# inkandswitch/peritext

Measured on NVIDIA H100. Metric: ops merged/sec across batch, higher is better.
Workload: dtype u32

## Files before the change

### peritext_b200/csrc/engine.cu

```cuda
#include <algorithm>
#include <atomic>
#include <cstdlib>
#include <cstring>
#include <initializer_list>
#include <string>
#include <thread>
#include <utility>
#include <vector>

#include "merge_kernel.cuh"
#include "warp_kernel.cuh"
#include "patch_kernel.cuh"
#include "patch_large_kernel.cuh"
#include "team_kernel.cuh"
#include "render_kernel.cuh"
#include "patch_json_kernel.cuh"
#include "append_kernel.cuh"
#include "change_kernel.cuh"
#include "exchange_kernel.cuh"
#include "changes_json_kernel.cuh"
#include "upload_kernel.cuh"
#include "scan_kernel.cuh"
#include "admit_kernel.cuh"
#include "query_kernel.cuh"
// ... 70 lines not shown
    uint64_t n_insdel = 0, n_mark = 0;
    std::vector<pt_log_desc> h_desc;
    ptp::Plan plan;
    DevBuf d_runs, d_tokens, d_run_off, d_tok_off, d_cins, d_cmarks;
    DevBuf d_desc, d_insdel, d_marks, d_order, d_counters, d_results, d_text_off, d_span_off, d_text, d_spans, d_pool, d_slab, d_retry, d_seq;
    DevBuf d_bsum, d_ctoff, d_csoff, d_ctext, d_cspans;
    DevBuf d_cdesc, d_changes, d_deps, d_admit;
    std::vector<pt_change_desc> h_cdesc;
    uint64_t n_changes = 0, n_deps = 0;
    DevBuf d_patch_recs, d_patch_items, d_patch_status;
    DevBuf d_patch_first;
    DevBuf d_large_cand, d_large_scratch;
    HostBuf h_patch_recs, h_patch_items, h_patch_status, h_patch_misc, h_patch_first;
    DevBuf d_jval, d_jvoff, d_jlink, d_jloff, d_jcom, d_jcoff;
    JsonBufs spans_json, patches_json;
    JsonBufs changes_json;
    HostBuf h_cj_status;
    DevBuf d_picnt, d_piseg, d_pibsum, d_pitmp, d_pisorted;
    uint64_t patch_cap = 0;
    bool have_changes = false;
    uint32_t adm_maxR = 1;
    const pt_insdel_rec* dp_insdel = nullptr;
    const pt_mark_rec* dp_marks = nullptr;
    DevBuf d_half_insdel, d_half_marks;
    HostBuf h_stage, h_results, h_text, h_spans, h_pool, h_misc, h_seq, h_ctoff, h_csoff;
    HostBuf h_chg_status, h_chg_desc, h_chg_insdel, h_chg_marks;
    HostBuf h_xch_totals, h_xch_status, h_xch_off, h_xch_delivered, h_xch_desc;
    bool have_actors = false;
    DevBuf d_anames, d_aoff, d_afirst;
    std::vector<uint64_t> h_afirst, h_abyte;
    std::vector<char> h_adense;
    HostBuf h_act_data, h_act_off, h_act_first;
    HostBuf h_syn_totals, h_syn_status, h_syn_off, h_syn_aoff, h_syn_amap;
    HostBuf h_add_totals, h_add_rank, h_add_aoff, h_add_amap;
    cudaEvent_t ev0 = nullptr, ev1 = nullptr;
    cudaStream_t side = nullptr, launch_stream = nullptr;
    cudaEvent_t ev_fork = nullptr, ev_join = nullptr;
    uint64_t launches = 0;
    cudaGraphExec_t graph_exec = nullptr;
    bool graph_ok = false, graph_tried = false;
    uint32_t merges_since_upload = 0;
    bool dl_begun = false;
    uint32_t kernels_per_merge = 0;
    uint64_t pool_used_host = 0;
};

namespace {
// ... 188 lines not shown
int install_plan(pt_batch* b, const pt_packed_ops& ops, ptp::Plan&& plan, bool own_records) {
    b->n_logs = ops.n_logs; b->n_insdel = ops.n_insdel_total; b->n_mark = ops.n_mark_total;
    b->h_desc.assign(ops.logs, ops.logs + ops.n_logs);
    b->plan = std::move(plan);
    int rc;
    if ((rc = alloc_and_upload_plan(b))) return rc;
    if (own_records) {
        if ((rc = reserve_n<pt_insdel_rec>(b->d_insdel, b->n_insdel))) return rc;
        if ((rc = reserve_n<pt_mark_rec>(b->d_marks, b->n_mark))) return rc;
    }
    return PT_OK;
}

int begin_upload(pt_batch* b, const pt_packed_ops& ops, bool own_records) {
    PT_CUDA(cudaSetDevice(b->device));
    PT_CUDA(cudaStreamSynchronize(b->stream));
    b->have_batch = false; b->merged = false; b->dl_begun = false; b->have_changes = false; b->have_actors = false;
    drop_graph(b);
    ptp::Plan plan;
    if (const char* err = ptp::make_plan(ops, b->limits, b->num_sms, plan)) { g_last_error = err; return PT_ERR_INVALID; }
    return install_plan(b, ops, std::move(plan), own_records);
}

int derive_half_records(pt_batch* b) {
    const uint32_t* nr = b->plan.n_route;
    if (!(nr[ptp::kPacked3] + nr[ptp::kCompact] + nr[ptp::kDirect])) { b->d_half_insdel.release(); b->d_half_marks.release(); return PT_OK; }
    int rc;
    if ((rc = reserve_n<uint2>(b->d_half_insdel, b->n_insdel)) || (rc = reserve_n<uint4>(b->d_half_marks, b->n_mark))) return rc;
    const uint64_t total = b->n_insdel + b->n_mark;
    const uint32_t threads = 256;
    if (total) {
        ptu::derive_half_records_kernel<<<warp_grid(b, total, threads, 1), threads, 0, b->stream>>>(
            b->dp_insdel, b->dp_marks, (uint2*)b->d_half_insdel.p, (uint4*)b->d_half_marks.p, b->n_insdel, b->n_mark);
        PT_CUDA(launched(b));
    }
    return PT_OK;
}

int finish_upload(pt_batch* b, const void* insdel, const void* marks, std::initializer_list<std::pair<const void*, uint64_t>> sources) {
    bool pageable = false;
    for (const auto& s : sources) {
        if (!s.second) continue;
        cudaPointerAttributes a;
        if (cudaPointerGetAttributes(&a, s.first) != cudaSuccess) { cudaGetLastError(); pageable = true; }
        else if (a.type != cudaMemoryTypeHost) pageable = true;
    }
    b->dp_insdel = (const pt_insdel_rec*)insdel; b->dp_marks = (const pt_mark_rec*)marks;
    int rc;
    if ((rc = derive_half_records(b))) return rc;
    if (pageable) PT_CUDA(cudaStreamSynchronize(b->stream));
    b->have_batch = true;
    return PT_OK;
}

template <class Q, class A, class Launch>
int run_queries(pt_batch* b, const char* fn, const char* verb, const Q* queries, uint32_t n, A* out, Launch launch) {
    if (!b || (n && (!queries || !out))) return PT_ERR_INVALID;
    if (!b->merged) { g_last_error = std::string(verb) + " before merge"; return PT_ERR_STATE; }
    if (!(b->limits.flags & PT_FLAG_EMIT_SEQUENCE)) { g_last_error = "the handle was created without PT_FLAG_EMIT_SEQUENCE"; return PT_ERR_STATE; }
    if (!n) return PT_OK;
    PT_CUDA(cudaSetDevice(b->device));
    DevBuf dq, da;
    int rc;
    if ((rc = dq.reserve((size_t)n * sizeof(Q))) || (rc = da.reserve((size_t)n * sizeof(A)))) return rc;
    cudaError_t e = cudaMemcpyAsync(dq.p, queries, (size_t)n * sizeof(Q), cudaMemcpyHostToDevice, b->stream);
    if (e == cudaSuccess) {
        launch(warp_grid(b, n, 128), 128u, (const Q*)dq.p, (A*)da.p);
        e = launched(b);
    }
    if (e == cudaSuccess) e = cudaMemcpyAsync(out, da.p, (size_t)n * sizeof(A), cudaMemcpyDeviceToHost, b->stream);
    if (e == cudaSuccess) e = cudaStreamSynchronize(b->stream);
    if (e != cudaSuccess) { g_last_error = std::string(fn) + ": " + cudaGetErrorString(e); return PT_ERR_CUDA; }
// ... 423 lines not shown
            pta::splice_changes_kernel<<<warp_grid(b, n, threads), threads, 0, b->stream>>>(
                (const pt_change_desc*)b->d_cdesc.p, (const pt_change_desc*)ncdesc.p, (const pt_change_desc*)dcdesc.p, n, DR,
                (const pt_change_rec*)b->d_changes.p, (const pt_dep_rec*)b->d_deps.p, d_dchg, d_ddep, (pt_change_rec*)nch.p, (pt_dep_rec*)ndp.p);
            PT_CUDA(launched(b));
        }
    }
    uint32_t bad = 0;
    PT_CUDA(cudaMemcpyAsync(&bad, abad.p, 4, cudaMemcpyDeviceToHost, b->stream));
    PT_CUDA(cudaStreamSynchronize(b->stream));
    if (bad) { g_last_error = std::string(fn) + "a resident comment rank is outside comment_map"; return PT_ERR_INVALID; }
    bool keep_actors = !(R.actor_off && R.actor_off[n] > R.actor_off[0]) && !(R.ctr_off && R.ctr_off[n] > R.ctr_off[0]);
    for (uint32_t i = 0; keep_actors && i < n; i++) keep_actors = nd[i].n_actors == b->h_desc[i].n_actors;
    b->have_actors = b->have_actors && keep_actors;
    b->have_batch = false; b->merged = false; b->dl_begun = false;
    drop_graph(b);
    b->d_insdel.swap(nins); b->d_marks.swap(nmarks);
    if (dch) {
        b->d_cdesc.swap(ncdesc); b->d_changes.swap(nch); b->d_deps.swap(ndp);
        b->h_cdesc = std::move(ncd); b->n_changes = n_ch; b->n_deps = n_dp; b->adm_maxR = maxR;
    }
    if ((rc = install_plan(b, ops, std::move(plan), true))) return rc;
    PT_CUDA(cudaStreamSynchronize(b->stream));
    b->dp_insdel = (const pt_insdel_rec*)b->d_insdel.p; b->dp_marks = (const pt_mark_rec*)b->d_marks.p;
    if ((rc = derive_half_records(b))) return rc;
    b->have_batch = true;
    return PT_OK;
}

int pt_batch_append(pt_batch* b, const pt_packed_ops* delta, const pt_append_remap* remap, const pt_change_table* dch) {
    if (!b || !delta || (delta->n_logs && !delta->logs)) return PT_ERR_INVALID;
    if (!b->have_batch) { g_last_error = "pt_batch_append before pt_batch_upload"; return PT_ERR_STATE; }
    return splice_append(b, "pt_batch_append: ", delta, false, remap ? *remap : pt_append_remap{}, dch, false);
}

static std::string check_change(const pt_batch* b, const pt_change_input& in, std::vector<pt_log_desc>& dd, std::vector<uint32_t>& new_elems,
                                std::vector<uint32_t>& work) {
    const uint32_t n = b->n_logs;
    if (in.n_logs != n) return "the input has " + std::to_string(in.n_logs) + " logs and the batch " + std::to_string(n);
    if (!n) return std::string();
    if (!in.actor || !in.input_off) return "null actor or input_off";
    if (in.input_off[0] != 0) return "input_off[0] is not 0";
    if ((in.input_off[n] && !in.ops) || (in.n_tokens && !in.tokens)) return "null ops or tokens with a nonzero count";
    dd.resize(n); new_elems.assign(n, 0);
    uint64_t io = 0, mo = 0;
    for (uint32_t i = 0; i < n; i++) {
        const pt_log_desc& L = b->h_desc[i];
        const uint64_t lo = in.input_off[i], hi = in.input_off[i + 1];
// ... 564 lines not shown
    } else {
        for (uint32_t i = 0; i < n; i++) tot[i] = pty::SyncTotals{};
    }
    if ((rc = grow_tables(b, fn, grow, tot, n, (const uint8_t*)ddata.p, (const unsigned long long*)doff.p, (const unsigned long long*)dfirst.p,
                          (const unsigned long long*)dnew.p, b->h_add_aoff, b->h_add_amap, &spliced))) return rc;
    if (count) {
        const pty::Tables T{(const uint8_t*)b->d_anames.p, (const unsigned long long*)b->d_aoff.p, (const unsigned long long*)b->d_afirst.p};
        pty::add_ranks_kernel<<<warp_grid(b, n, 128), 128, 0, b->stream>>>(n, T, (const uint8_t*)ddata.p, (const unsigned long long*)doff.p,
                                                                           (const unsigned long long*)dfirst.p, (uint16_t*)drank.p);
        PT_CUDA(launched(b));
        PT_CUDA(cudaMemcpyAsync(b->h_add_rank.p, drank.p, count * 2, cudaMemcpyDeviceToHost, b->stream));
        PT_CUDA(cudaStreamSynchronize(b->stream));
    }
    *out = pt_actor_view{n, count, (const uint16_t*)b->h_add_rank.p, (const uint64_t*)b->h_add_aoff.p, (const uint16_t*)b->h_add_amap.p, spliced ? 1u : 0u};
    return PT_OK;
}

static int enqueue_merge(pt_batch* b) {
    DevCounters* c = counters(b);
    PT_CUDA(cudaMemsetAsync(c, 0, sizeof(DevCounters), b->stream));
    ptk::BatchParams P{};
    P.desc = (const pt_log_desc*)b->d_desc.p;
    P.insdel = b->dp_insdel; P.marks = b->dp_marks;
    P.half_insdel = (const uint2*)b->d_half_insdel.p; P.half_marks = (const uint4*)b->d_half_marks.p;
    P.results = (pt_log_result*)b->d_results.p;
    P.text_off = (const uint64_t*)b->d_text_off.p; P.span_off = (const uint64_t*)b->d_span_off.p;
    P.text = (uint32_t*)b->d_text.p; P.spans = (pt_span*)b->d_spans.p;
    P.comment_pool = (uint32_t*)b->d_pool.p; P.comment_used = &c->comment_used; P.comment_cap = b->plan.pool_cap;
    P.slab = (char*)b->d_slab.p;
    P.slab_counter = c->slab; P.slab_slots = b->plan.slab_slots;
    P.seq = (b->limits.flags & PT_FLAG_EMIT_SEQUENCE) ? (uint32_t*)b->d_seq.p : nullptr;
    P.stats = c->stats;
    P.admit = nullptr;
    if (b->have_changes && b->n_logs) {
        const auto [wpb, smem] = actor_shape(b->adm_maxR);
        if (smem > 48 * 1024) PT_CUDA(cudaFuncSetAttribute(ptadm::admit_kernel, cudaFuncAttributeMaxDynamicSharedMemorySize, (int)smem));
        ptadm::admit_kernel<<<warp_grid(b, b->n_logs, wpb * 32), wpb * 32, smem, b->stream>>>(
            (const pt_change_desc*)b->d_cdesc.p, (const pt_change_rec*)b->d_changes.p, (const pt_dep_rec*)b->d_deps.p, (const pt_log_desc*)b->d_desc.p,
            b->n_logs, b->adm_maxR, (uint32_t*)b->d_admit.p, (pt_log_result*)b->d_results.p);
        PT_CUDA(launched(b));
        P.admit = (const uint32_t*)b->d_admit.p;
    }
    { const char* e = getenv("PT_PREFETCH"); P.prefetch_next = e ? (uint32_t)atoi(e) : 0u; }
    { const char* e = getenv("PT_WARP_FLAGS"); P.warp_flags = e ? (uint32_t)atoi(e) : 0x704u; }
    { const char* e = getenv("PT_TMA"); P.use_tma = e ? (uint32_t)atoi(e) : 1u; }
    int rc;
    const uint32_t* bin_first = b->plan.bin_first;
// ... 588 lines not shown
```

### peritext_b200/csrc/merge_kernel.cuh

```cuda
#pragma once
#include <cuda_runtime.h>
#include <stdint.h>

#include "../../include/peritext_b200.h"
#include "../../include/pt_digest.h"

namespace ptk {

struct BatchParams {
    const pt_log_desc* __restrict__ desc;
    const pt_insdel_rec* __restrict__ insdel;
    const pt_mark_rec* __restrict__ marks;
    const uint2* __restrict__ half_insdel;
    const uint4* __restrict__ half_marks;
    const uint32_t* __restrict__ order;
    uint32_t n_work;
    uint32_t* work_counter;
    pt_log_result* results;
    const uint64_t* __restrict__ text_off;
    const uint64_t* __restrict__ span_off;
    uint32_t* text;
    pt_span* spans;
    uint32_t* comment_pool;
    unsigned long long* comment_used;
    unsigned long long comment_cap;
    char* slab;
    unsigned long long slab_bytes;
    uint32_t* slab_counter;
    uint32_t slab_slots;
    uint32_t smem_arena_bytes;
    unsigned long long* stats;
    uint32_t* retry_list;
    uint32_t* retry_count;
    const uint32_t* n_work_dev;
    uint32_t prefetch_next;
    uint32_t warp_flags;
    uint32_t use_tma;
// ... 975 lines not shown
```

### peritext_b200/csrc/upload_kernel.cuh

```cuda
#pragma once
#include <cstdint>

#include "../../include/peritext_b200.h"

namespace ptu {

__global__ void expand_runs_kernel(const pt_log_desc* __restrict__ desc, const unsigned long long* __restrict__ run_off,
                                   const unsigned long long* __restrict__ tok_off, const pt_run_rec* __restrict__ runs,
                                   const uint32_t* __restrict__ tokens, pt_insdel_rec* __restrict__ out, uint32_t n_logs) {
    const uint32_t warp = (blockIdx.x * blockDim.x + threadIdx.x) >> 5, lane = threadIdx.x & 31, nwarps = (gridDim.x * blockDim.x) >> 5;
    for (uint32_t li = warp; li < n_logs; li += nwarps) {
        const unsigned long long r0 = run_off[li], r1 = run_off[li + 1];
        pt_insdel_rec* o = out + desc[li].insdel_off;
        const uint32_t* tk = tokens + tok_off[li];
        uint32_t rec_base = 0, tok_base = 0;
        for (unsigned long long rb = r0; rb < r1; rb += 32) {
            const unsigned long long ri = rb + lane;
            uint4 r = make_uint4(0, 0, 0, 0);
            uint32_t cnt = 0, kind = 0;
            if (ri < r1) { r = __ldg(reinterpret_cast<const uint4*>(runs + ri)); cnt = r.w & 0x3FFFFFFFu; kind = r.w >> 30; }
            uint32_t tcnt = kind == PT_KIND_INSERT ? cnt : 0u;
            uint32_t pr = cnt, pt = tcnt;
#pragma unroll
            for (int d = 1; d < 32; d <<= 1) { uint32_t a = __shfl_up_sync(0xffffffffu, pr, d), b2 = __shfl_up_sync(0xffffffffu, pt, d); if (lane >= (uint32_t)d) { pr += a; pt += b2; } }
// ... 21 lines not shown
    for (unsigned long long i = (unsigned long long)blockIdx.x * blockDim.x + threadIdx.x; i < n; i += (unsigned long long)gridDim.x * blockDim.x) {
        const uint2 q = __ldg(reinterpret_cast<const uint2*>(in + i));
        const uint32_t tok22 = q.y >> 10;
        uint4 o;
        o.x = q.x & 0xFFFFu; o.y = q.x >> 16;
        o.z = (q.y & 0xFu) | (((q.y >> 4) & 0xFu) << 16);
        o.w = (((q.y >> 8) & 3u) << 30) | ((tok22 & 0x200000u) ? PT_TOKEN_POOLED : 0u) | (tok22 & 0x1FFFFFu);
        reinterpret_cast<uint4*>(out)[i] = o;
    }
}
__global__ void expand_mark_c16_kernel(const pt_mark_c16* __restrict__ in, pt_mark_rec* __restrict__ out, unsigned long long n) {
    for (unsigned long long i = (unsigned long long)blockIdx.x * blockDim.x + threadIdx.x; i < n; i += (unsigned long long)gridDim.x * blockDim.x) {
        const uint4 q = __ldg(reinterpret_cast<const uint4*>(in + i));
        uint4 a, b;
        a.x = q.x & 0xFFFFu;
        a.y = (q.w & 0xFu) | (((q.w >> 12) & 7u) << 16) | (((q.w >> 15) & 0xFu) << 24);
        a.z = q.x >> 16; a.w = q.y & 0xFFFFu;
        b.x = ((q.w >> 4) & 0xFu) | (((q.w >> 8) & 0xFu) << 16);
        b.y = q.z; b.z = q.y >> 16; b.w = 0;
        reinterpret_cast<uint4*>(out)[2 * i] = a; reinterpret_cast<uint4*>(out)[2 * i + 1] = b;
    }
}

__device__ __forceinline__ uint32_t sat16(uint32_t v) { return min(v, 0xFFFFu); }
__device__ __forceinline__ uint32_t sat8(uint32_t v) { return min(v, 0xFFu); }
__global__ void derive_half_records_kernel(const pt_insdel_rec* __restrict__ ins, const pt_mark_rec* __restrict__ mk,
                                           uint2* __restrict__ hins, uint4* __restrict__ hmk, unsigned long long n, unsigned long long m) {
    for (unsigned long long i = (unsigned long long)blockIdx.x * blockDim.x + threadIdx.x; i < n + m; i += (unsigned long long)gridDim.x * blockDim.x) {
        if (i < n) {
            const uint4 r = __ldg(reinterpret_cast<const uint4*>(ins + i));
            hins[i] = make_uint2(sat16(r.x) | (sat16(r.y) << 16), sat8(r.z & 0xFFFFu) | (sat8(r.z >> 16) << 8) | ((r.w >> 30) << 16));
        } else {
            const uint4* q = reinterpret_cast<const uint4*>(mk + (i - n));
            const uint4 a = __ldg(q), b = __ldg(q + 1);
            hmk[i - n] = make_uint4(sat16(a.x) | (sat16(a.z) << 16), sat16(a.w) | (sat16(b.z) << 16), b.y,
                                    sat8(a.y & 0xFFFFu) | (sat8(b.x & 0xFFFFu) << 8) | (sat8(b.x >> 16) << 16) |
                                        (((a.y >> 16) & 7u) << 24) | (((a.y >> 24) & 0xFu) << 27));
        }
    }
}

}
```

### peritext_b200/csrc/warp_kernel.cuh

```cuda
#pragma once
#include "merge_kernel.cuh"

namespace ptk {

constexpr uint32_t kFull = 0xffffffffu;
constexpr uint32_t kNone16 = 0xFFFFu;
constexpr uint32_t kWarpGrab = 4;
constexpr uint32_t kMaxSegSurvivorWork = 1536;
constexpr uint32_t kMaxCommentSurvivors = 48;

__device__ __forceinline__ uint32_t warp_incl_scan(uint32_t v, uint32_t lane) {
#pragma unroll
    for (int o = 1; o < 32; o <<= 1) { const uint32_t y = __shfl_up_sync(kFull, v, o); if (lane >= (uint32_t)o) v += y; }
    return v;
}

struct WArena {
    uint32_t base, used, cap;
    template <class T> __device__ __forceinline__ T* alloc(uint32_t count) {
        const uint32_t off = used;
        used += (uint32_t)((count * sizeof(T) + 15u) & ~15u);
        return reinterpret_cast<T*>(ptk_smem + base + off);
    }
    __device__ __forceinline__ bool fits() const { return used <= cap; }
// ... 38 lines not shown
    __device__ __forceinline__ void mark(int k) { const long long now = clock64(); c[k] += (unsigned long long)(now - t); t = now; }
};
#define PT_PHASE(k) pclk.mark(k)
#define PT_PHASE_PARAM , PhaseClock& pclk
#define PT_PHASE_ARG , pclk
#else
#define PT_PHASE(k) ((void)0)
#define PT_PHASE_PARAM
#define PT_PHASE_ARG
#endif

constexpr int kIdDirect = 0, kIdCompact = 1, kIdPacked3 = 2;

template <int IDM>
__device__ __forceinline__ int warp_merge_one_log(const BatchParams& P, const uint32_t li, const uint32_t slice_base, const uint32_t slice_bytes, const uint32_t li_next, PhaseSync ps PT_PHASE_PARAM) {
    const uint32_t lane = threadIdx.x & 31u;
    const uint32_t lt = (1u << lane) - 1u;

    const uint4 dsc0 = __ldg(reinterpret_cast<const uint4*>(P.desc + li)), dsc1 = __ldg(reinterpret_cast<const uint4*>(P.desc + li) + 1);
    const unsigned long long insdel_off = (unsigned long long)dsc0.x | ((unsigned long long)dsc0.y << 32);
    const unsigned long long mark_off = (unsigned long long)dsc0.z | ((unsigned long long)dsc0.w << 32);
    const uint32_t n = dsc1.x, m = dsc1.y, R = dsc1.z ? dsc1.z : 1u, C = dsc1.w;
    const unsigned long long KS64 = (unsigned long long)C * R;
    if (KS64 >= 0xFFFFull || n >= 0xFFFFu || m >= 0xFFFFu || R > 255u) { ps.leave(); return 1; }
    const uint32_t KS = (uint32_t)KS64;
    const uint2* __restrict__ ins = P.half_insdel + insdel_off;
    const uint4* __restrict__ mk = P.half_marks + mark_off;
    const pt_insdel_rec* __restrict__ full_ins = P.insdel + insdel_off;
    uint32_t* text_out = P.text + P.text_off[li];
    pt_span* span_out = P.spans + P.span_off[li];
    pt_log_result* res = P.results + li;

    if ((P.warp_flags & 1u) && m) {
        const char* p0 = reinterpret_cast<const char*>(mk);
        const uint32_t lines = (m * 16u + 127u) >> 7;
        for (uint32_t l = lane; l < lines; l += 32) prefetch_l2(p0 + ((size_t)l << 7));
    }

    WArena A; A.base = slice_base; A.used = 0; A.cap = slice_bytes;
    uint32_t st = 0;
    auto keyOf = [&](uint32_t ctr, uint32_t actor) -> uint32_t { return (ctr - 1u) * R + actor; };
    auto badId = [&](uint32_t ctr, uint32_t actor) -> bool { return ctr - 1u >= C || actor >= R; };
    auto fail = [&](uint32_t code) { st |= 1u << code; };
    auto failDup = [&]() { st |= 1u; };
    auto bail = [&](uint32_t code) { if (lane == 0) { pt_log_result r{}; r.status = code; *res = r; } };

    constexpr bool compact = IDM == kIdCompact, packed = IDM == kIdPacked3;
    if (compact && !(R >= 3u && R <= 30u && n <= 2046u)) { ps.leave(); return 1; }
    if (packed && !(R == 3u && n <= 1022u)) { ps.leave(); return 1; }
    constexpr uint32_t kOvSlots = 128, kOvMax = 96, kOvEmpty = 0xFFFFFFFFu;
    const uint32_t NWr = (n + 31) / 32 + 1;
    uint32_t* OV = A.alloc<uint32_t>(compact ? kOvSlots : 0u);
    uint4* WI = A.alloc<uint4>(NWr);
    uint16_t* T = A.alloc<uint16_t>(packed ? 2u * C : compact ? C : KS);
    uint32_t* T32 = reinterpret_cast<uint32_t*>(T);
    if (!A.fits()) { ps.leave(); return 1; }
    if (packed) wfill<uint32_t>(T32, C, 0u, lane);
    else wfill<uint16_t>(T, compact ? C : KS, (uint16_t)kNone16, lane);
    if (compact) wfill<uint32_t>(OV, kOvSlots, kOvEmpty, lane);
    wfill<uint32_t>(reinterpret_cast<uint32_t*>(WI), 4 * NWr, 0u, lane);
    __syncwarp();
    auto ovHash = [&](uint32_t key) -> uint32_t { return ((key * 40503u) >> 7) & (kOvSlots - 1u); };
    auto lookup = [&](uint32_t ctr, uint32_t actor) -> uint32_t {
        if (packed) { const uint32_t f = (T32[ctr - 1u] >> (10u * actor)) & 1023u; return f ? f - 1u : kNone16; }
        if (!compact) return T[keyOf(ctr, actor)];
        const uint32_t e = T[ctr - 1u];
        if (e == kNone16) return kNone16;
        if ((e >> 11) == actor) return e & 0x7FFu;
        const uint32_t key = keyOf(ctr, actor);
        for (uint32_t h = ovHash(key);; h = (h + 1u) & (kOvSlots - 1u)) {
            const uint32_t v = OV[h];
            if (v == kOvEmpty) return kNone16;
            if ((v >> 16) == key) return v & 0xFFFFu;
        }
    };

    uint32_t nOv = 0;
    {
        uint32_t carryK = 0xFFFFFFFFu;
        const uint32_t nm1 = n ? n - 1u : 0u;
        uint2 ra = make_uint2(0, 0);
        if (n) ra = __ldg(ins + min(lane, nm1));
        const char* insb = reinterpret_cast<const char*>(ins);
        const uint32_t insBytes = n * 8u;
        if (lane * 128u + 512u < insBytes) prefetch_l2(insb + 512u + lane * 128u);
        PT_PHASE(kPhStart);
#pragma unroll 2
        for (uint32_t base = 0; base < n; base += 32) {
            const uint32_t i = base + lane;
            if ((base & 511u) == 0u) {
                const uint32_t po = (base + 576u) * 8u + lane * 128u;
                if (po < insBytes) prefetch_l2(insb + po);
            }
            const uint2 rc = __ldg(ins + min(i + 32u, nm1));
            const uint2 r = ra;
            const uint32_t ctr = r.x & 0xFFFFu, ref_ctr = r.x >> 16, actor = r.y & 0xFFu, ref_actor = (r.y >> 8) & 0xFFu, kind = r.y >> 16;
            const bool inb = i < n;
            const bool kbad = kind > 1u, ibad = badId(ctr, actor);
            const bool valid = inb && !kbad && !ibad;
            if (inb && kbad) fail(PT_LOG_BAD_KIND);
            if (inb && ibad) fail(PT_LOG_BAD_OPID);
            const uint32_t key = keyOf(ctr, actor);
            const bool isIns = valid && kind == PT_KIND_INSERT;
            bool toOv = false, wrote = false;
            uint32_t mine = 0;
            if (isIns) {
                if (packed) {
                    const uint32_t sh = 10u * actor;
                    if ((atomicOr(&T32[ctr - 1u], (i + 1u) << sh) >> sh) & 1023u) failDup();
                } else if (!compact) {
                    if (T[key] != kNone16) failDup();
                    T[key] = (uint16_t)i;
                } else {
                    mine = (actor << 11) | i;
                    const uint32_t e = T[ctr - 1u];
                    if (e == kNone16) { T[ctr - 1u] = (uint16_t)mine; wrote = true; }
                    else if ((e >> 11) == actor) failDup();
                    else toOv = true;
                }
            }
            const uint32_t myK = isIns ? key : 0xFFFFFFFFu;
            uint32_t prevK = __shfl_up_sync(kFull, myK, 1);
            if (lane == 0) prevK = carryK;
            carryK = __shfl_sync(kFull, myK, 31);
            const bool refOk = ref_ctr != 0 && !badId(ref_ctr, ref_actor);
            const uint32_t rkey = keyOf(ref_ctr, ref_actor);
            bool cand = isIns && refOk && rkey == prevK;
            if (cand && rkey >= key) { fail(PT_LOG_CYCLE); cand = false; }
            const uint32_t insW = __ballot_sync(kFull, isIns), candW = __ballot_sync(kFull, cand);
            if (lane == 0) *reinterpret_cast<uint2*>(&WI[base >> 5]) = make_uint2(insW, candW);
            __syncwarp();
            if (IDM == kIdDirect) {
                if (isIns && T[key] != (uint16_t)i) failDup();
            } else if (compact) {
                if (wrote) {
                    const uint32_t e2 = T[ctr - 1u];
                    if (e2 != mine) { if ((e2 >> 11) == actor) failDup(); else toOv = true; }
                }
                const uint32_t ovW = __ballot_sync(kFull, toOv);
                if (ovW) {
                    nOv += __popc(ovW);
                    if (toOv && nOv <= kOvMax) {
                        const uint32_t val = (key << 16) | i;
                        for (uint32_t h = ovHash(key);; h = (h + 1u) & (kOvSlots - 1u)) {
                            const uint32_t old = atomicCAS(&OV[h], kOvEmpty, val);
                            if (old == kOvEmpty) break;
                            if ((old >> 16) == key) { failDup(); break; }
                        }
                    }
                    __syncwarp();
                }
            }
            {
                const bool need = valid && !cand, hasRef = ref_ctr != 0;
                uint32_t j = kNone16;
                if (need && refOk) j = lookup(ref_ctr, ref_actor);
                const bool found = j != kNone16 && j < i;
                const bool cyc = isIns && rkey >= key;
                if (need) {
                    if (hasRef ? !found : !isIns) fail(PT_LOG_ELEM_NOT_FOUND);
                    else if (hasRef && cyc) fail(PT_LOG_CYCLE);
                }
                if (need && found && !cyc) atomicOr(reinterpret_cast<uint32_t*>(&WI[j >> 5]) + (isIns ? 2u : 3u), 1u << (j & 31));
            }
            ra = rc;
        }
    }
    __syncwarp();
    ps.pass();
    if (compact && nOv > kOvMax) { ps.leave(); return 1; }
    st = __reduce_or_sync(kFull, st);
    if (st) { bail(st > 1u ? 31u - __clz(st) : PT_LOG_BAD_OPID); ps.leave(); return 0; }
    PT_PHASE(kPhAB);

    uint32_t M, nvis, N = 0;
    {
        uint32_t carryH = 0, carryV = 0, otherCarry = 0;
        for (uint32_t wb = 0; wb < NWr; wb += 32) {
            const uint32_t w = wb + lane;
            uint32_t insW = 0, candW = 0, otherW = 0, delW = 0;
            if (w < NWr) { const uint4 q = WI[w]; insW = q.x; candW = q.y; otherW = q.z; delW = q.w; }
            const uint32_t up = __shfl_up_sync(kFull, otherW, 1);
            const uint32_t prevBit = lane ? (up >> 31) : otherCarry;
            otherCarry = __shfl_sync(kFull, otherW, 31) >> 31;
            const uint32_t head = insW & (~candW | ((otherW << 1) | prevBit));
            const uint32_t vis = insW & ~delW;
            const uint32_t pc = __popc(head) | (__popc(vis) << 16);
            const uint32_t inc = warp_incl_scan(pc, lane), ex = inc - pc, tot = __shfl_sync(kFull, inc, 31);
            if (w < NWr) WI[w] = make_uint4(insW, head, vis, (carryH + (ex & 0xFFFFu)) | ((carryV + (ex >> 16)) << 16));
            if (head & 0xFFFFu) prefetch_l2(ins + w * 32u);
            if (head >> 16) prefetch_l2(ins + w * 32u + 16u);
            carryH += tot & 0xFFFFu; carryV += tot >> 16;
            N += __reduce_add_sync(kFull, (uint32_t)__popc(insW));
        }
        M = carryH; nvis = carryV;
    }
    __syncwarp();
    PT_PHASE(kPhC);

    auto runOf = [&](uint32_t i) -> uint32_t {
        const uint4 q = WI[i >> 5];
        return (q.w & 0xFFFFu) + __popc(q.y & (0xFFFFFFFFu >> (31 - (i & 31)))) - 1u;
    };
    auto visBefore = [&](uint32_t i) -> uint32_t {
        const uint4 q = WI[i >> 5];
        return (q.w >> 16) + __popc(q.z & ((1u << (i & 31)) - 1u));
    };

    if ((P.warp_flags & 2u) && li_next != 0xFFFFFFFFu && lane == 0) prefetch_l2(P.desc + li_next);
    const uint32_t E = 2 * (M + 1), END = (E + 7u) & ~7u;
    if (END + 1 >= 0xFFFFu) { ps.leave(); return 1; }
    uint16_t* VisBase = A.alloc<uint16_t>(M + 1);
    const uint32_t markD = A.used;
    {
// ... 8 lines not shown
        const uint32_t uBytes = max((uint32_t)(((KW + 1) * 4 + 15) & ~15u) + (uint32_t)(((KW + 1) * 2 + 15) & ~15u), 2u * (uint32_t)((nSp * 4 + 15) & ~15u));
        char* U = A.alloc<char>(uBytes);
        if (!A.fits()) { ps.leave(); return 1; }
        uint32_t* KBits = reinterpret_cast<uint32_t*>(U);
        uint16_t* KPre = reinterpret_cast<uint16_t*>(U + (((KW + 1) * 4 + 15) & ~15u));
        uint32_t* Sub = reinterpret_cast<uint32_t*>(U);
        uint32_t* Sub2 = reinterpret_cast<uint32_t*>(U + ((nSp * 4 + 15) & ~15u));
#pragma unroll 1
        for (uint32_t wb = 0; wb < NWr; wb += 32) {
            const uint32_t w = wb + lane;
            if (w < NWr) {
                const uint4 q = WI[w];
                uint32_t hb = q.y, rid = q.w & 0xFFFFu;
                while (hb) { const uint32_t b = __ffs(hb) - 1; hb &= hb - 1; HV[rid++] = (uint16_t)(w * 32 + b); }
            }
        }
        wfill<uint32_t>(KBits, KW + 1, 0u, lane);
        __syncwarp();
#pragma unroll 1
        for (uint32_t rb = 0; rb < M; rb += 32) {
            const uint32_t r = rb + lane;
            if (r < M) {
                const uint32_t i = HV[r], w = i >> 5, b = i & 31;
                const uint2 rec = __ldg(ins + i);
                const uint4 q0 = WI[w];
                uint32_t stop = (q0.y | ~q0.x) & ~(0xFFFFFFFFu >> (31 - b));
                uint32_t ww = w;
                while (!stop) { ww++; const uint2 q1 = *reinterpret_cast<const uint2*>(&WI[ww]); stop = q1.y | ~q1.x; }
                const uint32_t end = ww * 32 + (__ffs(stop) - 1);
                const uint32_t key = keyOf(rec.x & 0xFFFFu, rec.y & 0xFFu), ref_ctr = rec.x >> 16;
                const uint32_t p = ref_ctr == 0 ? n : lookup(ref_ctr, (rec.y >> 8) & 0xFFu);
                const uint32_t q = p == n ? M : runOf(p);
                const uint32_t hv = visBefore(i);
                N16[2 * r + 1] = (uint16_t)(visBefore(end) - hv);
                HV[r] = (uint16_t)hv;
                Prun[r] = (uint16_t)q; RKey[r] = (uint16_t)key;
                atomicOr(&KBits[key >> 5], 1u << (key & 31));
            }
        }
        __syncwarp();
        {
            uint32_t carry = 0;
#pragma unroll 1
            for (uint32_t wb = 0; wb < KW; wb += 32) {
                const uint32_t w = wb + lane;
                const uint32_t cnt = w < KW ? __popc(KBits[w]) : 0u;
                const uint32_t inc = warp_incl_scan(cnt, lane);
                if (w < KW) KPre[w] = (uint16_t)(carry + inc - cnt);
                carry += __shfl_sync(kFull, inc, 31);
            }
        }
        __syncwarp();
#pragma unroll 1
        for (uint32_t rb = 0; rb < M; rb += 32) {
// ... 92 lines not shown
    for (uint32_t w = 0; w + 1 < NWr; w++) {
        const uint4 q = WI[w];
        const uint32_t ib = q.x;
        if (!ib) continue;
        const uint32_t hbits = q.y, vbits = q.z, hp = q.w & 0xFFFFu, vp = q.w >> 16;
        if ((ib >> lane) & 1u) {
            const uint32_t i = w * 32 + lane;
            const uint32_t run = hp + __popc(hbits & (0xFFFFFFFFu >> (31 - lane))) - 1u;
            const uint32_t vr = ((uint32_t)VisBase[run] + vp + __popc(vbits & lt)) & 0xFFFFu;
            const uint32_t isv = (vbits >> lane) & 1u;
            EV[i] = (uint16_t)(vr | (isv << 15));
            if (isv) {
                const uint32_t tok = PT_PAYLOAD_TOKEN(__ldg(&full_ins[i].payload));
                text_out[vr] = tok;
                digest_add(d0, d1, pt_term_text(vr, tok));
            }
        }
    }
    __syncwarp();

    uint32_t nspans = 0;
    if ((P.warp_flags & 2u) && li_next != 0xFFFFFFFFu) {
        const uint4 q0 = __ldg(reinterpret_cast<const uint4*>(P.desc + li_next)), q1 = __ldg(reinterpret_cast<const uint4*>(P.desc + li_next) + 1);
        const char* p0 = reinterpret_cast<const char*>(P.half_insdel + ((unsigned long long)q0.x | ((unsigned long long)q0.y << 32)));
        const uint32_t lines = (q1.x * 8u + 127u) >> 7;
        for (uint32_t l = lane; l < lines; l += 32) prefetch_l2(p0 + ((size_t)l << 7));
    }

    if (m) {
        const uint32_t pfb = min(m * 16u, 6u * 1024u);
        for (uint32_t o = lane * 128u; o < pfb; o += 32u * 128u) prefetch_l2(reinterpret_cast<const char*>(mk) + o);
    }
    PT_PHASE(kPhF);
    uint32_t nS = 0, nC = 0;
    uint4* Sv = nullptr;
    uint16_t* CIdx = nullptr;
    if (m) {
        const uint32_t KW = (KS + 31) / 32;
        uint32_t* KBits = A.alloc<uint32_t>(KW + 1);
        CIdx = A.alloc<uint16_t>(kMaxCommentSurvivors + 32);
        if (!A.fits()) { ps.leave(); return 1; }
        const uint32_t room = A.cap - A.used, svStart = A.used;
        uint32_t capS = room > 256u ? (room - 256u) / 16u : 0u;
        if (capS > m) capS = m;
        Sv = A.alloc<uint4>(capS + 1);
        if (!A.fits()) { ps.leave(); return 1; }
        wfill<uint32_t>(KBits, KW + 1, 0u, lane);
        __syncwarp();
        const uint32_t mm1 = m - 1u;
        uint4 a = __ldg(mk + min(lane, mm1));
        const uint32_t mkBytes = m * 16u;
#pragma unroll 2
        for (uint32_t kb = 0; kb < m; kb += 32) {
            const uint32_t k = kb + lane;
            if ((kb & 255u) == 0u) {
                const uint32_t po = (kb + 384u) * 16u + lane * 128u;
                if (po < mkBytes) prefetch_l2(reinterpret_cast<const char*>(mk) + po);
            }
            const uint4 b = __ldg(mk + min(k + 32u, mm1));
            const uint32_t ctr = a.x & 0xFFFFu, start_ctr = a.x >> 16, end_ctr = a.y & 0xFFFFu, arrival = a.y >> 16, attr = a.z;
            const uint32_t actor = a.w & 0xFFu, start_actor = (a.w >> 8) & 0xFFu, end_actor = (a.w >> 16) & 0xFFu, kind = (a.w >> 24) & 7u, bounds = a.w >> 27;
            const uint32_t type = (kind >> 1) & 3u;
            const bool inb = k < m;
            const bool idok = inb && !badId(ctr, actor);
            const uint32_t key = keyOf(ctr, actor);
            bool dup = false;
            if (idok) {
                const uint32_t bit = 1u << (key & 31);
                dup = (atomicOr(&KBits[key >> 5], bit) & bit) != 0 || lookup(ctr, actor) != kNone16;
            }
            if (inb && (!idok || dup)) fail(PT_LOG_BAD_OPID);
            const uint32_t sb = bounds & 3u, eb = (bounds >> 2) & 3u;
            const bool sOk = idok && sb <= PT_BOUND_AFTER && !badId(start_ctr, start_actor);
            uint32_t js = kNone16;
            if (sOk) js = lookup(start_ctr, start_actor);
            const bool sHit = js != kNone16 && js < arrival;
            uint32_t es = 0;
            if (sHit) es = EV[js];
            const uint32_t va = (es & 0x7FFFu) + (sb & (es >> 15));
            const bool eOk = sHit && eb <= PT_BOUND_AFTER && !badId(end_ctr, end_actor);
            uint32_t je = kNone16;
            if (eOk) je = lookup(end_ctr, end_actor);
            const bool eHit = je != kNone16 && je < arrival && !(je == js && eb == sb);
            uint32_t vb = nvis;
            if (eHit) { const uint32_t ee = EV[je]; vb = (ee & 0x7FFFu) + (eb & (ee >> 15)); }
            const bool surv = sHit && va < vb;
            const bool isC = surv && type == PT_MARK_COMMENT;
            const uint32_t bal = __ballot_sync(kFull, surv), balC = __ballot_sync(kFull, isC);
            if (surv) {
                const uint32_t idx = nS + __popc(bal & lt);
                if (idx < capS) {
                    Sv[idx] = make_uint4(va | (vb << 16), (type == PT_MARK_COMMENT ? k : key) | (kind << 16), attr, 0u);
                    if (isC) { const uint32_t ci = nC + __popc(balC & lt); if (ci <= kMaxCommentSurvivors) CIdx[ci] = (uint16_t)idx; }
                }
            }
            nS += __popc(bal); nC += __popc(balC);
            a = b;
        }
        __syncwarp();
        st = __reduce_or_sync(kFull, st);
        if (st) { bail(31u - __clz(st)); ps.leave(); return 0; }
        if (nS > capS) { ps.leave(); return 1; }
        A.used = svStart + ((nS * 16u + 15u) & ~15u);
    }

    ps.pass();
    PT_PHASE(kPhG);
    unsigned long long pool_base = 0;
    if (nvis == 0) nspans = 0;
    else if (nS == 0) {
        if (lane == 0) {
            pt_span s; s.start = 0; s.flags = 0; s.link_attr = PT_ATTR_NONE; s.comment_off = 0;
            span_out[0] = s;
            digest_add(d0, d1, pt_term_span(0, 0, 0, PT_ATTR_NONE));
        }
        nspans = 1;
    } else {
        if (nC > kMaxCommentSurvivors) { ps.leave(); return 1; }
        if (nvis <= 32u && nC <= 32u) {
            const uint32_t x = lane;
            uint32_t w0 = 0, w1 = 0, w2 = 0, flags = 0, link = PT_ATTR_NONE;
#pragma unroll 1
            for (uint32_t j = 0; j < nS; j++) {
                const uint4 sv = Sv[j];
                const uint32_t ab = sv.x, pk = sv.y;
                const bool cover = x >= (ab & 0xFFFFu) && x < (ab >> 16);
// ... 324 lines not shown
```

Before: 97.76 billion.

## Precompute packed op keys at upload to shrink per-merge record reads

At upload, a per-log pass now converts each insert/delete record into a single 32-bit pair of precomputed op keys, and each mark into an 8-byte record holding keys, arrival, kind and bounds. This replaces the old 8- and 16-byte half records. The warp merge kernel reads these smaller records directly, so it no longer recomputes keys or validates ids, and the lookup takes a key, recovering the counter with a reciprocal multiply. Mark attributes are dropped from the hot record and fetched afterwards from the full records, only for surviving link and comment marks. The change also tightens the fallback limit (n>2047 when marks exist) and adds divide-by-multiply work inside lookups.

```diff
diff --git a/peritext_b200/csrc/engine.cu b/peritext_b200/csrc/engine.cu
--- a/peritext_b200/csrc/engine.cu
+++ b/peritext_b200/csrc/engine.cu
@@ -116,7 +116,7 @@
     uint32_t adm_maxR = 1;
     const pt_insdel_rec* dp_insdel = nullptr;
     const pt_mark_rec* dp_marks = nullptr;
-    DevBuf d_half_insdel, d_half_marks;
+    DevBuf d_key_insdel, d_key_marks;
     HostBuf h_stage, h_results, h_text, h_spans, h_pool, h_misc, h_seq, h_ctoff, h_csoff;
     HostBuf h_chg_status, h_chg_desc, h_chg_insdel, h_chg_marks;
     HostBuf h_xch_totals, h_xch_status, h_xch_off, h_xch_delivered, h_xch_desc;
@@ -351,16 +351,15 @@
     return install_plan(b, ops, std::move(plan), own_records);
 }
 
-int derive_half_records(pt_batch* b) {
+int derive_key_records(pt_batch* b) {
     const uint32_t* nr = b->plan.n_route;
-    if (!(nr[ptp::kPacked3] + nr[ptp::kCompact] + nr[ptp::kDirect])) { b->d_half_insdel.release(); b->d_half_marks.release(); return PT_OK; }
-    int rc;
-    if ((rc = reserve_n<uint2>(b->d_half_insdel, b->n_insdel)) || (rc = reserve_n<uint4>(b->d_half_marks, b->n_mark))) return rc;
-    const uint64_t total = b->n_insdel + b->n_mark;
+    if (!(nr[ptp::kPacked3] + nr[ptp::kCompact] + nr[ptp::kDirect])) { b->d_key_insdel.release(); b->d_key_marks.release(); return PT_OK; }
+    int rc;
+    if ((rc = reserve_n<uint32_t>(b->d_key_insdel, b->n_insdel)) || (rc = reserve_n<uint2>(b->d_key_marks, b->n_mark))) return rc;
     const uint32_t threads = 256;
-    if (total) {
-        ptu::derive_half_records_kernel<<<warp_grid(b, total, threads, 1), threads, 0, b->stream>>>(
-            b->dp_insdel, b->dp_marks, (uint2*)b->d_half_insdel.p, (uint4*)b->d_half_marks.p, b->n_insdel, b->n_mark);
+    if (b->n_logs) {
+        ptu::derive_key_records_kernel<<<warp_grid(b, b->n_logs, threads), threads, 0, b->stream>>>(
+            (const pt_log_desc*)b->d_desc.p, b->dp_insdel, b->dp_marks, (uint32_t*)b->d_key_insdel.p, (uint2*)b->d_key_marks.p, b->n_logs);
         PT_CUDA(launched(b));
     }
     return PT_OK;
@@ -376,7 +375,7 @@
     }
     b->dp_insdel = (const pt_insdel_rec*)insdel; b->dp_marks = (const pt_mark_rec*)marks;
     int rc;
-    if ((rc = derive_half_records(b))) return rc;
+    if ((rc = derive_key_records(b))) return rc;
     if (pageable) PT_CUDA(cudaStreamSynchronize(b->stream));
     b->have_batch = true;
     return PT_OK;
@@ -846,7 +845,7 @@
     if ((rc = install_plan(b, ops, std::move(plan), true))) return rc;
     PT_CUDA(cudaStreamSynchronize(b->stream));
     b->dp_insdel = (const pt_insdel_rec*)b->d_insdel.p; b->dp_marks = (const pt_mark_rec*)b->d_marks.p;
-    if ((rc = derive_half_records(b))) return rc;
+    if ((rc = derive_key_records(b))) return rc;
     b->have_batch = true;
     return PT_OK;
 }
@@ -1457,7 +1456,7 @@
     ptk::BatchParams P{};
     P.desc = (const pt_log_desc*)b->d_desc.p;
     P.insdel = b->dp_insdel; P.marks = b->dp_marks;
-    P.half_insdel = (const uint2*)b->d_half_insdel.p; P.half_marks = (const uint4*)b->d_half_marks.p;
+    P.key_insdel = (const uint32_t*)b->d_key_insdel.p; P.key_marks = (const uint2*)b->d_key_marks.p;
     P.results = (pt_log_result*)b->d_results.p;
     P.text_off = (const uint64_t*)b->d_text_off.p; P.span_off = (const uint64_t*)b->d_span_off.p;
     P.text = (uint32_t*)b->d_text.p; P.spans = (pt_span*)b->d_spans.p;
diff --git a/peritext_b200/csrc/merge_kernel.cuh b/peritext_b200/csrc/merge_kernel.cuh
--- a/peritext_b200/csrc/merge_kernel.cuh
+++ b/peritext_b200/csrc/merge_kernel.cuh
@@ -11,8 +11,8 @@
     const pt_log_desc* __restrict__ desc;
     const pt_insdel_rec* __restrict__ insdel;
     const pt_mark_rec* __restrict__ marks;
-    const uint2* __restrict__ half_insdel;
-    const uint4* __restrict__ half_marks;
+    const uint32_t* __restrict__ key_insdel;
+    const uint2* __restrict__ key_marks;
     const uint32_t* __restrict__ order;
     uint32_t n_work;
     uint32_t* work_counter;
diff --git a/peritext_b200/csrc/upload_kernel.cuh b/peritext_b200/csrc/upload_kernel.cuh
--- a/peritext_b200/csrc/upload_kernel.cuh
+++ b/peritext_b200/csrc/upload_kernel.cuh
@@ -67,20 +67,40 @@
     }
 }
 
-__device__ __forceinline__ uint32_t sat16(uint32_t v) { return min(v, 0xFFFFu); }
-__device__ __forceinline__ uint32_t sat8(uint32_t v) { return min(v, 0xFFu); }
-__global__ void derive_half_records_kernel(const pt_insdel_rec* __restrict__ ins, const pt_mark_rec* __restrict__ mk,
-                                           uint2* __restrict__ hins, uint4* __restrict__ hmk, unsigned long long n, unsigned long long m) {
-    for (unsigned long long i = (unsigned long long)blockIdx.x * blockDim.x + threadIdx.x; i < n + m; i += (unsigned long long)gridDim.x * blockDim.x) {
-        if (i < n) {
-            const uint4 r = __ldg(reinterpret_cast<const uint4*>(ins + i));
-            hins[i] = make_uint2(sat16(r.x) | (sat16(r.y) << 16), sat8(r.z & 0xFFFFu) | (sat8(r.z >> 16) << 8) | ((r.w >> 30) << 16));
-        } else {
-            const uint4* q = reinterpret_cast<const uint4*>(mk + (i - n));
+constexpr uint32_t kKeyS0 = 0xFFFEu, kKeyS1 = 0xFFFFu;
+__global__ void derive_key_records_kernel(const pt_log_desc* __restrict__ desc, const pt_insdel_rec* __restrict__ ins,
+                                          const pt_mark_rec* __restrict__ mk, uint32_t* __restrict__ kins, uint2* __restrict__ kmk,
+                                          uint32_t n_logs) {
+    const uint32_t warp = (blockIdx.x * blockDim.x + threadIdx.x) >> 5, lane = threadIdx.x & 31, nwarps = (gridDim.x * blockDim.x) >> 5;
+    for (uint32_t li = warp; li < n_logs; li += nwarps) {
+        const uint4 d0 = __ldg(reinterpret_cast<const uint4*>(desc + li)), d1 = __ldg(reinterpret_cast<const uint4*>(desc + li) + 1);
+        const uint32_t n = d1.x, m = d1.y, R = d1.z ? d1.z : 1u, C = d1.w;
+        if ((unsigned long long)C * R >= 0xFFFFull) continue;
+        const unsigned long long io = (unsigned long long)d0.x | ((unsigned long long)d0.y << 32);
+        const unsigned long long mo = (unsigned long long)d0.z | ((unsigned long long)d0.w << 32);
+        auto key = [&](uint32_t c, uint32_t a) -> uint32_t { return c - 1u < C && a < R ? (c - 1u) * R + a : kKeyS1; };
+        for (uint32_t i = lane; i < n; i += 32) {
+            const uint4 r = __ldg(reinterpret_cast<const uint4*>(ins + io + i));
+            const uint32_t kind = r.w >> 30;
+            uint32_t own = kind > 1u ? kKeyS1 : key(r.x, r.z & 0xFFFFu), ref = kKeyS1;
+            if (kind <= 1u) {
+                if (own == kKeyS1) ref = kKeyS0;
+                else {
+                    if (kind == PT_KIND_DELETE) own = kKeyS0;
+                    ref = r.y == 0 ? kKeyS0 : key(r.y, r.z >> 16);
+                }
+            }
+            kins[io + i] = own | (ref << 16);
+        }
+        const uint32_t narr = min(n, 0x7FFu);
+        for (uint32_t k = lane; k < m; k += 32) {
+            const uint4* q = reinterpret_cast<const uint4*>(mk + mo + k);
             const uint4 a = __ldg(q), b = __ldg(q + 1);
-            hmk[i - n] = make_uint4(sat16(a.x) | (sat16(a.z) << 16), sat16(a.w) | (sat16(b.z) << 16), b.y,
-                                    sat8(a.y & 0xFFFFu) | (sat8(b.x & 0xFFFFu) << 8) | (sat8(b.x >> 16) << 16) |
-                                        (((a.y >> 16) & 7u) << 24) | (((a.y >> 24) & 0xFu) << 27));
+            const uint32_t sb = (a.y >> 24) & 3u, eb = (a.y >> 26) & 3u;
+            const uint32_t s = sb <= PT_BOUND_AFTER ? key(a.z, b.x & 0xFFFFu) : kKeyS1, e = eb <= PT_BOUND_AFTER ? key(a.w, b.x >> 16) : kKeyS1;
+            kmk[mo + k] = make_uint2(key(a.x, a.y & 0xFFFFu) | (s << 16),
+                                     e | (min(b.z, narr) << 16) | (((a.y >> 16) & 7u) << 27) |
+                                         ((sb <= PT_BOUND_AFTER ? sb : 0u) << 30) | ((eb <= PT_BOUND_AFTER ? eb : 0u) << 31));
         }
     }
 }
diff --git a/peritext_b200/csrc/warp_kernel.cuh b/peritext_b200/csrc/warp_kernel.cuh
--- a/peritext_b200/csrc/warp_kernel.cuh
+++ b/peritext_b200/csrc/warp_kernel.cuh
@@ -1,5 +1,6 @@
 #pragma once
 #include "merge_kernel.cuh"
+#include "upload_kernel.cuh"
 
 namespace ptk {
 
@@ -84,10 +85,11 @@
     const unsigned long long mark_off = (unsigned long long)dsc0.z | ((unsigned long long)dsc0.w << 32);
     const uint32_t n = dsc1.x, m = dsc1.y, R = dsc1.z ? dsc1.z : 1u, C = dsc1.w;
     const unsigned long long KS64 = (unsigned long long)C * R;
-    if (KS64 >= 0xFFFFull || n >= 0xFFFFu || m >= 0xFFFFu || R > 255u) { ps.leave(); return 1; }
+    if (KS64 >= 0xFFFFull || n >= 0xFFFFu || m >= 0xFFFFu || (m && n > 2047u)) { ps.leave(); return 1; }
     const uint32_t KS = (uint32_t)KS64;
-    const uint2* __restrict__ ins = P.half_insdel + insdel_off;
-    const uint4* __restrict__ mk = P.half_marks + mark_off;
+    constexpr uint32_t kS0 = ptu::kKeyS0, kS1 = ptu::kKeyS1;
+    const uint32_t* __restrict__ ins = P.key_insdel + insdel_off;
+    const uint2* __restrict__ mk = P.key_marks + mark_off;
     const pt_insdel_rec* __restrict__ full_ins = P.insdel + insdel_off;
     uint32_t* text_out = P.text + P.text_off[li];
     pt_span* span_out = P.spans + P.span_off[li];
@@ -95,14 +97,12 @@
 
     if ((P.warp_flags & 1u) && m) {
         const char* p0 = reinterpret_cast<const char*>(mk);
-        const uint32_t lines = (m * 16u + 127u) >> 7;
+        const uint32_t lines = (m * 8u + 127u) >> 7;
         for (uint32_t l = lane; l < lines; l += 32) prefetch_l2(p0 + ((size_t)l << 7));
     }
 
     WArena A; A.base = slice_base; A.used = 0; A.cap = slice_bytes;
     uint32_t st = 0;
-    auto keyOf = [&](uint32_t ctr, uint32_t actor) -> uint32_t { return (ctr - 1u) * R + actor; };
-    auto badId = [&](uint32_t ctr, uint32_t actor) -> bool { return ctr - 1u >= C || actor >= R; };
     auto fail = [&](uint32_t code) { st |= 1u << code; };
     auto failDup = [&]() { st |= 1u; };
     auto bail = [&](uint32_t code) { if (lane == 0) { pt_log_result r{}; r.status = code; *res = r; } };
@@ -123,13 +123,15 @@
     wfill<uint32_t>(reinterpret_cast<uint32_t*>(WI), 4 * NWr, 0u, lane);
     __syncwarp();
     auto ovHash = [&](uint32_t key) -> uint32_t { return ((key * 40503u) >> 7) & (kOvSlots - 1u); };
-    auto lookup = [&](uint32_t ctr, uint32_t actor) -> uint32_t {
-        if (packed) { const uint32_t f = (T32[ctr - 1u] >> (10u * actor)) & 1023u; return f ? f - 1u : kNone16; }
-        if (!compact) return T[keyOf(ctr, actor)];
-        const uint32_t e = T[ctr - 1u];
+    const uint32_t invR = compact ? 0xFFFFFFFFu / R + 1u : 0u;
+    auto ctrOf = [&](uint32_t key) -> uint32_t { return packed ? (key * 0xAAABu) >> 17 : __umulhi(key, invR); };
+    auto lookup = [&](uint32_t key) -> uint32_t {
+        if (!packed && !compact) return T[key];
+        const uint32_t c = ctrOf(key), actor = key - c * (packed ? 3u : R);
+        if (packed) { const uint32_t f = (T32[c] >> (10u * actor)) & 1023u; return f ? f - 1u : kNone16; }
+        const uint32_t e = T[c];
         if (e == kNone16) return kNone16;
         if ((e >> 11) == actor) return e & 0x7FFu;
-        const uint32_t key = keyOf(ctr, actor);
         for (uint32_t h = ovHash(key);; h = (h + 1u) & (kOvSlots - 1u)) {
             const uint32_t v = OV[h];
             if (v == kOvEmpty) return kNone16;
@@ -141,42 +143,36 @@
     {
         uint32_t carryK = 0xFFFFFFFFu;
         const uint32_t nm1 = n ? n - 1u : 0u;
-        uint2 ra = make_uint2(0, 0);
+        uint32_t ra = 0;
         if (n) ra = __ldg(ins + min(lane, nm1));
         const char* insb = reinterpret_cast<const char*>(ins);
-        const uint32_t insBytes = n * 8u;
-        if (lane * 128u + 512u < insBytes) prefetch_l2(insb + 512u + lane * 128u);
+        const uint32_t insBytes = n * 4u;
+        for (uint32_t o = 256u + lane * 128u; o < insBytes; o += 32u * 128u) prefetch_l2(insb + o);
         PT_PHASE(kPhStart);
 #pragma unroll 2
         for (uint32_t base = 0; base < n; base += 32) {
             const uint32_t i = base + lane;
-            if ((base & 511u) == 0u) {
-                const uint32_t po = (base + 576u) * 8u + lane * 128u;
-                if (po < insBytes) prefetch_l2(insb + po);
-            }
-            const uint2 rc = __ldg(ins + min(i + 32u, nm1));
-            const uint2 r = ra;
-            const uint32_t ctr = r.x & 0xFFFFu, ref_ctr = r.x >> 16, actor = r.y & 0xFFu, ref_actor = (r.y >> 8) & 0xFFu, kind = r.y >> 16;
+            const uint32_t rc = __ldg(ins + min(i + 32u, nm1));
+            const uint32_t own = ra & 0xFFFFu, rkey = ra >> 16;
             const bool inb = i < n;
-            const bool kbad = kind > 1u, ibad = badId(ctr, actor);
-            const bool valid = inb && !kbad && !ibad;
-            if (inb && kbad) fail(PT_LOG_BAD_KIND);
-            if (inb && ibad) fail(PT_LOG_BAD_OPID);
-            const uint32_t key = keyOf(ctr, actor);
-            const bool isIns = valid && kind == PT_KIND_INSERT;
+            const bool valid = inb && own != kS1;
+            if (inb && !valid) fail(rkey == kS1 ? PT_LOG_BAD_KIND : PT_LOG_BAD_OPID);
+            const uint32_t key = own;
+            const bool isIns = valid && own != kS0;
             bool toOv = false, wrote = false;
             uint32_t mine = 0;
             if (isIns) {
                 if (packed) {
-                    const uint32_t sh = 10u * actor;
-                    if ((atomicOr(&T32[ctr - 1u], (i + 1u) << sh) >> sh) & 1023u) failDup();
+                    const uint32_t c = ctrOf(key), sh = 10u * (key - 3u * c);
+                    if ((atomicOr(&T32[c], (i + 1u) << sh) >> sh) & 1023u) failDup();
                 } else if (!compact) {
                     if (T[key] != kNone16) failDup();
                     T[key] = (uint16_t)i;
                 } else {
+                    const uint32_t c = ctrOf(key), actor = key - c * R;
                     mine = (actor << 11) | i;
-                    const uint32_t e = T[ctr - 1u];
-                    if (e == kNone16) { T[ctr - 1u] = (uint16_t)mine; wrote = true; }
+                    const uint32_t e = T[c];
+                    if (e == kNone16) { T[c] = (uint16_t)mine; wrote = true; }
                     else if ((e >> 11) == actor) failDup();
                     else toOv = true;
                 }
@@ -185,8 +181,7 @@
             uint32_t prevK = __shfl_up_sync(kFull, myK, 1);
             if (lane == 0) prevK = carryK;
             carryK = __shfl_sync(kFull, myK, 31);
-            const bool refOk = ref_ctr != 0 && !badId(ref_ctr, ref_actor);
-            const uint32_t rkey = keyOf(ref_ctr, ref_actor);
+            const bool refOk = rkey < kS0;
             bool cand = isIns && refOk && rkey == prevK;
             if (cand && rkey >= key) { fail(PT_LOG_CYCLE); cand = false; }
             const uint32_t insW = __ballot_sync(kFull, isIns), candW = __ballot_sync(kFull, cand);
@@ -196,8 +191,8 @@
                 if (isIns && T[key] != (uint16_t)i) failDup();
             } else if (compact) {
                 if (wrote) {
-                    const uint32_t e2 = T[ctr - 1u];
-                    if (e2 != mine) { if ((e2 >> 11) == actor) failDup(); else toOv = true; }
+                    const uint32_t e2 = T[ctrOf(key)];
+                    if (e2 != mine) { if ((e2 >> 11) == (mine >> 11)) failDup(); else toOv = true; }
                 }
                 const uint32_t ovW = __ballot_sync(kFull, toOv);
                 if (ovW) {
@@ -214,9 +209,9 @@
                 }
             }
             {
-                const bool need = valid && !cand, hasRef = ref_ctr != 0;
+                const bool need = valid && !cand, hasRef = rkey != kS0;
                 uint32_t j = kNone16;
-                if (need && refOk) j = lookup(ref_ctr, ref_actor);
+                if (need && refOk) j = lookup(rkey);
                 const bool found = j != kNone16 && j < i;
                 const bool cyc = isIns && rkey >= key;
                 if (need) {
@@ -250,8 +245,7 @@
             const uint32_t pc = __popc(head) | (__popc(vis) << 16);
             const uint32_t inc = warp_incl_scan(pc, lane), ex = inc - pc, tot = __shfl_sync(kFull, inc, 31);
             if (w < NWr) WI[w] = make_uint4(insW, head, vis, (carryH + (ex & 0xFFFFu)) | ((carryV + (ex >> 16)) << 16));
-            if (head & 0xFFFFu) prefetch_l2(ins + w * 32u);
-            if (head >> 16) prefetch_l2(ins + w * 32u + 16u);
+            if (head) prefetch_l2(ins + w * 32u);
             carryH += tot & 0xFFFFu; carryV += tot >> 16;
             N += __reduce_add_sync(kFull, (uint32_t)__popc(insW));
         }
@@ -306,14 +300,14 @@
             const uint32_t r = rb + lane;
             if (r < M) {
                 const uint32_t i = HV[r], w = i >> 5, b = i & 31;
-                const uint2 rec = __ldg(ins + i);
+                const uint32_t rec = __ldg(ins + i);
                 const uint4 q0 = WI[w];
                 uint32_t stop = (q0.y | ~q0.x) & ~(0xFFFFFFFFu >> (31 - b));
                 uint32_t ww = w;
                 while (!stop) { ww++; const uint2 q1 = *reinterpret_cast<const uint2*>(&WI[ww]); stop = q1.y | ~q1.x; }
                 const uint32_t end = ww * 32 + (__ffs(stop) - 1);
-                const uint32_t key = keyOf(rec.x & 0xFFFFu, rec.y & 0xFFu), ref_ctr = rec.x >> 16;
-                const uint32_t p = ref_ctr == 0 ? n : lookup(ref_ctr, (rec.y >> 8) & 0xFFu);
+                const uint32_t key = rec & 0xFFFFu, rkey = rec >> 16;
+                const uint32_t p = rkey == kS0 ? n : lookup(rkey);
                 const uint32_t q = p == n ? M : runOf(p);
                 const uint32_t hv = visBefore(i);
                 N16[2 * r + 1] = (uint16_t)(visBefore(end) - hv);
@@ -452,13 +446,13 @@
     uint32_t nspans = 0;
     if ((P.warp_flags & 2u) && li_next != 0xFFFFFFFFu) {
         const uint4 q0 = __ldg(reinterpret_cast<const uint4*>(P.desc + li_next)), q1 = __ldg(reinterpret_cast<const uint4*>(P.desc + li_next) + 1);
-        const char* p0 = reinterpret_cast<const char*>(P.half_insdel + ((unsigned long long)q0.x | ((unsigned long long)q0.y << 32)));
-        const uint32_t lines = (q1.x * 8u + 127u) >> 7;
+        const char* p0 = reinterpret_cast<const char*>(P.key_insdel + ((unsigned long long)q0.x | ((unsigned long long)q0.y << 32)));
+        const uint32_t lines = (q1.x * 4u + 127u) >> 7;
         for (uint32_t l = lane; l < lines; l += 32) prefetch_l2(p0 + ((size_t)l << 7));
     }
 
     if (m) {
-        const uint32_t pfb = min(m * 16u, 6u * 1024u);
+        const uint32_t pfb = min(m * 8u, 6u * 1024u);
         for (uint32_t o = lane * 128u; o < pfb; o += 32u * 128u) prefetch_l2(reinterpret_cast<const char*>(mk) + o);
     }
     PT_PHASE(kPhF);
@@ -478,39 +472,37 @@
         wfill<uint32_t>(KBits, KW + 1, 0u, lane);
         __syncwarp();
         const uint32_t mm1 = m - 1u;
-        uint4 a = __ldg(mk + min(lane, mm1));
-        const uint32_t mkBytes = m * 16u;
+        uint2 a = __ldg(mk + min(lane, mm1));
+        const uint32_t mkBytes = m * 8u;
 #pragma unroll 2
         for (uint32_t kb = 0; kb < m; kb += 32) {
             const uint32_t k = kb + lane;
-            if ((kb & 255u) == 0u) {
-                const uint32_t po = (kb + 384u) * 16u + lane * 128u;
+            if ((kb & 511u) == 0u) {
+                const uint32_t po = (kb + 768u) * 8u + lane * 128u;
                 if (po < mkBytes) prefetch_l2(reinterpret_cast<const char*>(mk) + po);
             }
-            const uint4 b = __ldg(mk + min(k + 32u, mm1));
-            const uint32_t ctr = a.x & 0xFFFFu, start_ctr = a.x >> 16, end_ctr = a.y & 0xFFFFu, arrival = a.y >> 16, attr = a.z;
-            const uint32_t actor = a.w & 0xFFu, start_actor = (a.w >> 8) & 0xFFu, end_actor = (a.w >> 16) & 0xFFu, kind = (a.w >> 24) & 7u, bounds = a.w >> 27;
+            const uint2 b = __ldg(mk + min(k + 32u, mm1));
+            const uint32_t key = a.x & 0xFFFFu, skey = a.x >> 16, ekey = a.y & 0xFFFFu, arrival = (a.y >> 16) & 0x7FFu;
+            const uint32_t kind = (a.y >> 27) & 7u, sb = (a.y >> 30) & 1u, eb = a.y >> 31;
             const uint32_t type = (kind >> 1) & 3u;
             const bool inb = k < m;
-            const bool idok = inb && !badId(ctr, actor);
-            const uint32_t key = keyOf(ctr, actor);
+            const bool idok = inb && key != kS1;
             bool dup = false;
             if (idok) {
                 const uint32_t bit = 1u << (key & 31);
-                dup = (atomicOr(&KBits[key >> 5], bit) & bit) != 0 || lookup(ctr, actor) != kNone16;
+                dup = (atomicOr(&KBits[key >> 5], bit) & bit) != 0 || lookup(key) != kNone16;
             }
             if (inb && (!idok || dup)) fail(PT_LOG_BAD_OPID);
-            const uint32_t sb = bounds & 3u, eb = (bounds >> 2) & 3u;
-            const bool sOk = idok && sb <= PT_BOUND_AFTER && !badId(start_ctr, start_actor);
+            const bool sOk = idok && skey != kS1;
             uint32_t js = kNone16;
-            if (sOk) js = lookup(start_ctr, start_actor);
+            if (sOk) js = lookup(skey);
             const bool sHit = js != kNone16 && js < arrival;
             uint32_t es = 0;
             if (sHit) es = EV[js];
             const uint32_t va = (es & 0x7FFFu) + (sb & (es >> 15));
-            const bool eOk = sHit && eb <= PT_BOUND_AFTER && !badId(end_ctr, end_actor);
+            const bool eOk = sHit && ekey != kS1;
             uint32_t je = kNone16;
-            if (eOk) je = lookup(end_ctr, end_actor);
+            if (eOk) je = lookup(ekey);
             const bool eHit = je != kNone16 && je < arrival && !(je == js && eb == sb);
             uint32_t vb = nvis;
             if (eHit) { const uint32_t ee = EV[je]; vb = (ee & 0x7FFFu) + (eb & (ee >> 15)); }
@@ -520,7 +512,7 @@
             if (surv) {
                 const uint32_t idx = nS + __popc(bal & lt);
                 if (idx < capS) {
-                    Sv[idx] = make_uint4(va | (vb << 16), (type == PT_MARK_COMMENT ? k : key) | (kind << 16), attr, 0u);
+                    Sv[idx] = make_uint4(va | (vb << 16), (type == PT_MARK_COMMENT ? k : key) | (kind << 16), PT_ATTR_NONE, k);
                     if (isC) { const uint32_t ci = nC + __popc(balC & lt); if (ci <= kMaxCommentSurvivors) CIdx[ci] = (uint16_t)idx; }
                 }
             }
@@ -532,6 +524,14 @@
         if (st) { bail(31u - __clz(st)); ps.leave(); return 0; }
         if (nS > capS) { ps.leave(); return 1; }
         A.used = svStart + ((nS * 16u + 15u) & ~15u);
+        const pt_mark_rec* __restrict__ full_mk = P.marks + (mk - P.key_marks);
+#pragma unroll 1
+        for (uint32_t s = lane; s < nS; s += 32) {
+            const uint4 sv = Sv[s];
+            const uint32_t t = (sv.y >> 17) & 3u;
+            if (t == PT_MARK_LINK || t == PT_MARK_COMMENT) Sv[s].z = __ldg(&full_mk[sv.w].attr);
+        }
+        __syncwarp();
     }
 
     ps.pass();
```

Result: faster. 101.5 billion, median of 6 (+3.9%).
